# speedinghzl/CCNet

Measured on NVIDIA H100. Metric: cca_fwd_bwd_pixels_per_s, higher is better.
Workload: dtype f32

## Files before the change

### ccnet_b200/csrc/cca_tc_stats.cuh

```cuda
#pragma once
#include "cca_items.cuh"
#include "cca_tc_common.cuh"

namespace cca {
namespace tc {

struct StatsParams {
    ItemSpace sp;
    int Cq;
    long npix;
    float *parts;
    uint8_t *zero_ptr;
    long zero_bytes;
    unsigned int *counters;
    int n_counters;
};

template <int LK, typename E> struct StatsSmem {
    using T = Tiles<LK, E>;
    static constexpr int kNS = (200 * 1024) / (2 * T::kSlot) < 4 ? (200 * 1024) / (2 * T::kSlot) : 4;
    static constexpr int off_ld = 0;
    static constexpr int off_tail = off_ld + kNS * 2 * T::kSlot;
    static constexpr int off_bar = off_tail + (128 - LK) * 128 + 1024;
    static constexpr int kBytes = off_bar + 8 * 2 * kNS;
    static_assert(kNS >= 2, "ring depth");
    static_assert(kBytes <= 232448, "shared memory budget");
};

template <int LK, typename E>
__global__ void __launch_bounds__(kThreads, 1)
cca_tc_stats_kernel(const __grid_constant__ CUtensorMap mqc, const __grid_constant__ CUtensorMap mqr,
                    const __grid_constant__ CUtensorMap mkc, const __grid_constant__ CUtensorMap mkr, StatsParams p)
{
    using T = Tiles<LK, E>;
    using S = StatsSmem<LK, E>;
    constexpr bool H16 = kH16<E>, F16 = kF16<E>;
    constexpr int kNS = S::kNS;
    constexpr int TERMS = H16 ? 1 : 3;
    extern __shared__ __align__(1024) uint8_t smem[];
    uint64_t *full = reinterpret_cast<uint64_t *>(smem + S::off_bar), *empty = full + kNS;
    const int tid = threadIdx.x, warp = tid >> 5, lane = tid & 31;
    const int KQ = p.Cq / 16;
    const int nk = p.sp.total > (int)blockIdx.x ? (p.sp.total - (int)blockIdx.x + (int)gridDim.x - 1) / (int)gridDim.x : 0;
    auto item_of = [&](int k) { return decode_item(p.sp, (int)blockIdx.x + k * (int)gridDim.x); };

    if (tid == 0) {
        for (int i = 0; i < kNS; ++i) { mbar_init(&full[i], 1); mbar_init(&empty[i], kConsumers); }
        fence_mbar_init();
        prefetch_tmap(&mqc); prefetch_tmap(&mqr); prefetch_tmap(&mkc); prefetch_tmap(&mkr);
    }
    __syncthreads();
    pdl_launch_dependents();

    if (warp == 0) {
        if (lane == 0) {
            for (int k = 0; k < nk; ++k) {
                const Item it = item_of(k);
                const int slot = k % kNS;
                mbar_wait(&empty[slot], ((k / kNS) & 1) ^ 1);
                uint8_t *dst = smem + S::off_ld + slot * 2 * T::kSlot;
                mbar_expect_tx(&full[slot], 2 * T::kSlot);
                for (int t = 0; t < 2; ++t) {
                    const CUtensorMap *m = t == 0 ? (it.col ? &mqc : &mqr) : (it.col ? &mkc : &mkr);
                    const int start = t == 0 ? it.q0 : it.k0;
                    const int cw = it.col ? it.line : start, ch = it.col ? start : it.line;
                    tma_load_4d(dst + t * T::kSlot, m, &full[slot], 0, cw, ch, it.b);
                    if constexpr (!H16) tma_load_4d(dst + t * T::kSlot + T::kTile, m, &full[slot], 32, cw, ch, it.b);
                }
            }
        }
    } else if (tid >= 128) {
        const int t = tid - 128, wg = t >> 7, wq = (t >> 5) & 3;
        {
            const long n16 = p.zero_bytes / 16;
            const long per = (n16 + gridDim.x - 1) / gridDim.x;
            const long lo = per * blockIdx.x, hi = lo + per < n16 ? lo + per : n16;
            uint4 *dst = reinterpret_cast<uint4 *>(p.zero_ptr);
            for (long i = lo + t; i < hi; i += kConsumers) dst[i] = make_uint4(0, 0, 0, 0);
            if (blockIdx.x == 0)
                for (int i = t; i < p.n_counters; i += kConsumers) p.counters[i] = 0u;
        }
        const uint32_t ld_base = smem_u32(smem + S::off_ld);
        for (int k = 0; k < nk; ++k) {
            const Item it = item_of(k);
            const int slot = k % kNS;
            mbar_wait(&full[slot], (k / kNS) & 1);
            uint8_t *qs = smem + S::off_ld + slot * 2 * T::kSlot;
            if constexpr (!H16) {
                convert_slot<LK, E>(qs, t);
                convert_slot<LK, E>(qs + T::kSlot, t);
            }
            const uint32_t qb = ld_base + slot * 2 * T::kSlot, kb = qb + T::kSlot;
            float acc[LK / 2];
            wg_fence();
            for (int ks = 0; ks < KQ; ++ks) {
                wgmma_ss<LK, F16>(acc, desc_kmaj<LK, E>(qb, 64 * wg, ks, false), desc_kmaj<LK, E>(kb, 0, ks, false), ks > 0, 0, 0);
                if constexpr (TERMS == 3) {
                    wgmma_ss<LK, F16>(acc, desc_kmaj<LK, E>(qb, 64 * wg, ks, false), desc_kmaj<LK, E>(kb, 0, ks, true), 1, 0, 0);
                    wgmma_ss<LK, F16>(acc, desc_kmaj<LK, E>(qb, 64 * wg, ks, true), desc_kmaj<LK, E>(kb, 0, ks, false), 1, 0, 0);
                }
            }
            wg_commit();
            wg_wait<0>();
            wg_acc_fence<LK / 2>(acc);
            mbar_arrive(&empty[slot]);
#pragma unroll
            for (int h = 0; h < 2; ++h) {
                const int r = 64 * wg + 16 * wq + (lane >> 2) + 8 * h;
                const int self = it.col ? it.q0 + r - it.k0 : -1;
                float m = -INFINITY;
#pragma unroll
                for (int j = 0; j < LK / 8; ++j)
#pragma unroll
                    for (int e = 0; e < 2; ++e) {
                        const int c = 8 * j + 2 * (lane & 3) + e;
                        if (c < it.lk && c != self) m = fmaxf(m, acc[4 * j + 2 * h + e]);
                    }
                m = fmaxf(m, __shfl_xor_sync(0xffffffffu, m, 1));
                m = fmaxf(m, __shfl_xor_sync(0xffffffffu, m, 2));
                const float nm = m == -INFINITY ? 0.f : -m * kLog2e;
                float l = 0.f;
#pragma unroll
                for (int j = 0; j < LK / 8; ++j)
#pragma unroll
                    for (int e = 0; e < 2; ++e) {
                        const int c = 8 * j + 2 * (lane & 3) + e;
                        if (c < it.lk && c != self) l += exp2f(fmaf(acc[4 * j + 2 * h + e], kLog2e, nm));
                    }
                l += __shfl_xor_sync(0xffffffffu, l, 1);
                l += __shfl_xor_sync(0xffffffffu, l, 2);
                if ((lane & 3) == 0 && r < it.lq)
                    p.parts[(long)part_index(p.sp, it) * p.npix + item_pixel(p.sp, it, r)] = l > 0.f ? m * kLog2e + log2f(l) : -INFINITY;
            }
        }
    }
}

struct StatsArgs {
    const void *q, *k;
    float *parts;
    unsigned int *counters;
    int n_counters;
    Dims d;
    cudaStream_t st;
    const char **why;
};

template <int LK, typename E> cudaError_t launch_stats(const StatsArgs &a)
{
    CUtensorMap m[4];
    const Dims &d = a.d;
    if (cudaError_t e = get_maps(m, {{a.q, d.B, d.Cq, LK, LK}, {a.k, d.B, d.Cq, LK, LK}}, d, kDtype<E>, a.why)) return e;
    StatsParams p;
    p.sp = make_space(d.B, d.H, d.W);
    p.Cq = d.Cq;
    p.npix = (long)d.B * d.H * d.W;
    p.parts = a.parts;
    p.zero_ptr = nullptr; p.zero_bytes = 0;
    p.counters = a.counters; p.n_counters = a.n_counters;
    return launch_kernel(cca_tc_stats_kernel<LK, E>, item_grid(p.sp), kThreads, StatsSmem<LK, E>::kBytes, false, a.st, m[0], m[1],
                         m[2], m[3], p);
}

extern template cudaError_t launch_stats<80, __half>(const StatsArgs &);
extern template cudaError_t launch_stats<112, __half>(const StatsArgs &);

}
}
```

Baseline: 40.47 million.

## Split stats items across consumer warpgroups with per-warpgroup stage pairs

Instead of both consumer warpgroups cooperating on each item (each computing 64 rows), each warpgroup now takes alternate items and computes all 128 rows in two wgmma passes. The ring is fixed at four stages, two per warpgroup, and the fp32 split conversion uses a per-warpgroup named barrier rather than all consumers. The goal is to remove cross-warpgroup synchronization and let one warpgroup's softmax stats overlap the other's MMA. The risk is more serialized work per item, and the fixed four-stage ring may not fit shared memory for some tile sizes.

```diff
diff --git a/ccnet_b200/csrc/cca_tc_stats.cuh b/ccnet_b200/csrc/cca_tc_stats.cuh
--- a/ccnet_b200/csrc/cca_tc_stats.cuh
+++ b/ccnet_b200/csrc/cca_tc_stats.cuh
@@ -18,14 +18,85 @@
 
 template <int LK, typename E> struct StatsSmem {
     using T = Tiles<LK, E>;
-    static constexpr int kNS = (200 * 1024) / (2 * T::kSlot) < 4 ? (200 * 1024) / (2 * T::kSlot) : 4;
+    static constexpr int kNS = 4;
     static constexpr int off_ld = 0;
     static constexpr int off_tail = off_ld + kNS * 2 * T::kSlot;
-    static constexpr int off_bar = off_tail + (128 - LK) * 128 + 1024;
+    static constexpr int off_bar = off_tail + (128 - LK) * 128;
     static constexpr int kBytes = off_bar + 8 * 2 * kNS;
-    static_assert(kNS >= 2, "ring depth");
+    static_assert(kNS == 4, "two stages per consumer warpgroup");
     static_assert(kBytes <= 232448, "shared memory budget");
 };
+
+template <int LK>
+__device__ __forceinline__ void stats_rows(const float (&acc)[LK / 2], const ItemSpace &sp, const Item &it, long npix, float *parts,
+                                           int r0, int lane)
+{
+#pragma unroll
+    for (int h = 0; h < 2; ++h) {
+        const int r = r0 + 8 * h;
+        const int self = it.col ? it.q0 + r - it.k0 : -1;
+        float m = -INFINITY;
+#pragma unroll
+        for (int j = 0; j < LK / 8; ++j)
+#pragma unroll
+            for (int e = 0; e < 2; ++e) {
+                const int c = 8 * j + 2 * (lane & 3) + e;
+                if (c < it.lk && c != self) m = fmaxf(m, acc[4 * j + 2 * h + e]);
+            }
+        m = fmaxf(m, __shfl_xor_sync(0xffffffffu, m, 1));
+        m = fmaxf(m, __shfl_xor_sync(0xffffffffu, m, 2));
+        const float nm = m == -INFINITY ? 0.f : -m * kLog2e;
+        float l = 0.f;
+#pragma unroll
+        for (int j = 0; j < LK / 8; ++j)
+#pragma unroll
+            for (int e = 0; e < 2; ++e) {
+                const int c = 8 * j + 2 * (lane & 3) + e;
+                if (c < it.lk && c != self) l += exp2f(fmaf(acc[4 * j + 2 * h + e], kLog2e, nm));
+            }
+        l += __shfl_xor_sync(0xffffffffu, l, 1);
+        l += __shfl_xor_sync(0xffffffffu, l, 2);
+        if ((lane & 3) == 0 && r < it.lq)
+            parts[(long)part_index(sp, it) * npix + item_pixel(sp, it, r)] = l > 0.f ? m * kLog2e + log2f(l) : -INFINITY;
+    }
+}
+
+constexpr int kBarStats = 3;
+
+template <int LK>
+__device__ __forceinline__ void convert_slot_wg(uint8_t *slot, int r, int bar)
+{
+    using T = Tiles<LK, float>;
+    const int rr = r < LK ? r : LK - 1, sw = rr & 7;
+    float4 raw[16];
+#pragma unroll
+    for (int bx = 0; bx < 2; ++bx)
+#pragma unroll
+        for (int hq = 0; hq < 2; ++hq)
+#pragma unroll
+            for (int j = 0; j < 4; ++j)
+                raw[8 * bx + 4 * hq + j] = *reinterpret_cast<const float4 *>(slot + bx * T::kTile + rr * 128 + (((hq * 4 + j) ^ sw) * 16));
+    named_bar_sync(bar, 128);
+    if (r < LK) {
+#pragma unroll
+        for (int bx = 0; bx < 2; ++bx)
+#pragma unroll
+            for (int hq = 0; hq < 2; ++hq) {
+                uint8_t *d = slot + bx * T::kTile + r * 16 + hq * 2 * T::kPStride;
+#pragma unroll
+                for (int j = 0; j < 2; ++j) {
+                    const float4 a = raw[8 * bx + 4 * hq + 2 * j], b = raw[8 * bx + 4 * hq + 2 * j + 1];
+                    const float v[8] = {a.x, a.y, a.z, a.w, b.x, b.y, b.z, b.w};
+                    uint4 hi, lo;
+                    split8(v, hi, lo);
+                    *reinterpret_cast<uint4 *>(d + j * T::kPStride) = hi;
+                    *reinterpret_cast<uint4 *>(d + j * T::kPStride + T::kLoOff) = lo;
+                }
+            }
+    }
+    fence_proxy_async();
+    named_bar_sync(bar, 128);
+}
 
 template <int LK, typename E>
 __global__ void __launch_bounds__(kThreads, 1)
@@ -44,8 +115,10 @@
     const int nk = p.sp.total > (int)blockIdx.x ? (p.sp.total - (int)blockIdx.x + (int)gridDim.x - 1) / (int)gridDim.x : 0;
     auto item_of = [&](int k) { return decode_item(p.sp, (int)blockIdx.x + k * (int)gridDim.x); };
 
+    auto stage_of = [](int k) { return (k & 1) + 2 * ((k >> 1) & 1); };
+
     if (tid == 0) {
-        for (int i = 0; i < kNS; ++i) { mbar_init(&full[i], 1); mbar_init(&empty[i], kConsumers); }
+        for (int i = 0; i < kNS; ++i) { mbar_init(&full[i], 1); mbar_init(&empty[i], 128); }
         fence_mbar_init();
         prefetch_tmap(&mqc); prefetch_tmap(&mqr); prefetch_tmap(&mkc); prefetch_tmap(&mkr);
     }
@@ -56,8 +129,8 @@
         if (lane == 0) {
             for (int k = 0; k < nk; ++k) {
                 const Item it = item_of(k);
-                const int slot = k % kNS;
-                mbar_wait(&empty[slot], ((k / kNS) & 1) ^ 1);
+                const int slot = stage_of(k);
+                mbar_wait(&empty[slot], ((k >> 2) & 1) ^ 1);
                 uint8_t *dst = smem + S::off_ld + slot * 2 * T::kSlot;
                 mbar_expect_tx(&full[slot], 2 * T::kSlot);
                 for (int t = 0; t < 2; ++t) {
@@ -70,7 +143,7 @@
             }
         }
     } else if (tid >= 128) {
-        const int t = tid - 128, wg = t >> 7, wq = (t >> 5) & 3;
+        const int t = tid - 128, wg = t >> 7, wq = (t >> 5) & 3, r = t & 127;
         {
             const long n16 = p.zero_bytes / 16;
             const long per = (n16 + gridDim.x - 1) / gridDim.x;
@@ -81,56 +154,32 @@
                 for (int i = t; i < p.n_counters; i += kConsumers) p.counters[i] = 0u;
         }
         const uint32_t ld_base = smem_u32(smem + S::off_ld);
-        for (int k = 0; k < nk; ++k) {
+        for (int k = wg; k < nk; k += 2) {
             const Item it = item_of(k);
-            const int slot = k % kNS;
-            mbar_wait(&full[slot], (k / kNS) & 1);
+            const int slot = stage_of(k);
+            mbar_wait(&full[slot], (k >> 2) & 1);
             uint8_t *qs = smem + S::off_ld + slot * 2 * T::kSlot;
             if constexpr (!H16) {
-                convert_slot<LK, E>(qs, t);
-                convert_slot<LK, E>(qs + T::kSlot, t);
+                convert_slot_wg<LK>(qs, r, kBarStats + wg);
+                convert_slot_wg<LK>(qs + T::kSlot, r, kBarStats + wg);
             }
             const uint32_t qb = ld_base + slot * 2 * T::kSlot, kb = qb + T::kSlot;
-            float acc[LK / 2];
-            wg_fence();
-            for (int ks = 0; ks < KQ; ++ks) {
-                wgmma_ss<LK, F16>(acc, desc_kmaj<LK, E>(qb, 64 * wg, ks, false), desc_kmaj<LK, E>(kb, 0, ks, false), ks > 0, 0, 0);
-                if constexpr (TERMS == 3) {
-                    wgmma_ss<LK, F16>(acc, desc_kmaj<LK, E>(qb, 64 * wg, ks, false), desc_kmaj<LK, E>(kb, 0, ks, true), 1, 0, 0);
-                    wgmma_ss<LK, F16>(acc, desc_kmaj<LK, E>(qb, 64 * wg, ks, true), desc_kmaj<LK, E>(kb, 0, ks, false), 1, 0, 0);
+#pragma unroll 1
+            for (int rb = 0; rb < 2; ++rb) {
+                float acc[LK / 2];
+                wg_fence();
+                for (int ks = 0; ks < KQ; ++ks) {
+                    wgmma_ss<LK, F16>(acc, desc_kmaj<LK, E>(qb, 64 * rb, ks, false), desc_kmaj<LK, E>(kb, 0, ks, false), ks > 0, 0, 0);
+                    if constexpr (TERMS == 3) {
+                        wgmma_ss<LK, F16>(acc, desc_kmaj<LK, E>(qb, 64 * rb, ks, false), desc_kmaj<LK, E>(kb, 0, ks, true), 1, 0, 0);
+                        wgmma_ss<LK, F16>(acc, desc_kmaj<LK, E>(qb, 64 * rb, ks, true), desc_kmaj<LK, E>(kb, 0, ks, false), 1, 0, 0);
+                    }
                 }
-            }
-            wg_commit();
-            wg_wait<0>();
-            wg_acc_fence<LK / 2>(acc);
-            mbar_arrive(&empty[slot]);
-#pragma unroll
-            for (int h = 0; h < 2; ++h) {
-                const int r = 64 * wg + 16 * wq + (lane >> 2) + 8 * h;
-                const int self = it.col ? it.q0 + r - it.k0 : -1;
-                float m = -INFINITY;
-#pragma unroll
-                for (int j = 0; j < LK / 8; ++j)
-#pragma unroll
-                    for (int e = 0; e < 2; ++e) {
-                        const int c = 8 * j + 2 * (lane & 3) + e;
-                        if (c < it.lk && c != self) m = fmaxf(m, acc[4 * j + 2 * h + e]);
-                    }
-                m = fmaxf(m, __shfl_xor_sync(0xffffffffu, m, 1));
-                m = fmaxf(m, __shfl_xor_sync(0xffffffffu, m, 2));
-                const float nm = m == -INFINITY ? 0.f : -m * kLog2e;
-                float l = 0.f;
-#pragma unroll
-                for (int j = 0; j < LK / 8; ++j)
-#pragma unroll
-                    for (int e = 0; e < 2; ++e) {
-                        const int c = 8 * j + 2 * (lane & 3) + e;
-                        if (c < it.lk && c != self) l += exp2f(fmaf(acc[4 * j + 2 * h + e], kLog2e, nm));
-                    }
-                l += __shfl_xor_sync(0xffffffffu, l, 1);
-                l += __shfl_xor_sync(0xffffffffu, l, 2);
-                if ((lane & 3) == 0 && r < it.lq)
-                    p.parts[(long)part_index(p.sp, it) * p.npix + item_pixel(p.sp, it, r)] = l > 0.f ? m * kLog2e + log2f(l) : -INFINITY;
+                wg_commit();
+                wg_wait<0>();
+                wg_acc_fence<LK / 2>(acc);
+                if (rb == 1) mbar_arrive(&empty[slot]);
+                stats_rows<LK>(acc, p.sp, it, p.npix, p.parts, 64 * rb + 16 * wq + (lane >> 2), lane);
             }
         }
     }
```

Result: no change. 40.38 million (median of 6 runs) (-0.2%).
